# imulki/serenade

Hardware: AMD Instinct MI355X
Metric: mel frames/sec converted (UNet ODE + vocoder), 80x1024 (higher is better)
Workload: dtype f32

## Files before the change

### serenade_amd/csrc/resunit_f32.hip

```cpp
#include <hip/hip_runtime.h>

#include "common.h"
#include "conv_common.h"
#include "fastdiv.h"
#include "serenade_hip.h"

namespace {

constexpr int NTH = 512;

template <int C_>
struct UCfg {
  static constexpr int C = C_, CH = C / 32;
  static constexpr int BMI = C == 32 ? 256 : 128;
  static constexpr int A_ROWS = BMI + SRN_RESUNIT_HALO_MAX + 2;
  static constexpr int A_PLANE = A_ROWS * 144;
  static constexpr int A_BYTES = CH * A_PLANE;
  static constexpr int UNIT = C * 144;
  static constexpr int G = 9216 / UNIT >= 2 ? 2 : 1;
  static constexpr int STAGE = G * UNIT;
  static constexpr int SMEM = A_BYTES + 2 * STAGE;
  static constexpr int F4R = C / 4, RSTEP = NTH / F4R;
  static constexpr int A_LD = (A_ROWS * F4R + NTH - 1) / NTH;
  static_assert(G * C * 8 == NTH, "one 16-B weight piece per thread per stage");
};

template <class R>
__global__ __launch_bounds__(NTH, 4) void resunit_f32_kernel(const SrnResUnitParams p, const int tiles_per_z,
                                                             const int n_tiles, const FDiv d_tpz) {
  constexpr int C = R::C, CH = R::CH, BMI = R::BMI, G = R::G;
  extern __shared__ __attribute__((aligned(16))) unsigned char smem_u[];
  unsigned char* const sA = smem_u;
  unsigned char* const sW = smem_u + R::A_BYTES;

  const int tid = threadIdx.x;
  const int lane = tid & 63;
  const int wave = __builtin_amdgcn_readfirstlane(tid >> 6);
  const int li = lane & 31;
  const int lh = lane >> 5;
  const int k = p.k, dil = p.dilation, T = p.T;
  const int p2 = (k - 1) / 2, p1 = p2 * dil;
  const int BMo = BMI - (k - 1);
  const int hr = BMI + (k - 1) * dil;
  const int U = k * CH;
  const int S = (U + G - 1) / G;
  const float slope = p.slope;

  const int w_n = (tid % (C * 8)) >> 3;
  const int w_g = tid / (C * 8);
  const int w_voff = w_n * (k * C * 4) + w_g * 128 + (tid & 7) * 16;
  const int w_dst = (w_g * C + w_n) * 144 + (tid & 7) * 16;
  const int w_bytes = C * k * C * 4;
  const __amdgpu_buffer_rsrc_t rs_w1 = srn_buffer_rsrc(p.w1, w_bytes);
  const __amdgpu_buffer_rsrc_t rs_w2 = srn_buffer_rsrc(p.w2, w_bytes);
  u32x4 wr;
  auto w_load = [&](const int j) {
    if (j >= S) wr = __builtin_amdgcn_raw_buffer_load_b128(rs_w2, w_voff, (j - S) * G * 128, 0);
    else wr = __builtin_amdgcn_raw_buffer_load_b128(rs_w1, w_voff, j * G * 128, 0);
  };
  auto w_store = [&](const int buf) {
    *reinterpret_cast<u32x4*>(sW + buf * R::STAGE + w_dst) = wr;
  };

  constexpr int A_LD = R::A_LD, F4R = R::F4R, RSTEP = R::RSTEP;
  const int a_f4 = tid % F4R;
  const int a_r0 = tid / F4R;
  const int a_voff = (a_r0 * C + a_f4 * 4) * 4;
  const int a_dst0 = (a_f4 >> 3) * R::A_PLANE + a_r0 * 144 + (a_f4 & 7) * 16;
  u32x4 pa[A_LD];
  auto load_a = [&](const int tile) {
    const int z = fdiv(tile, d_tpz);
    const int t0 = (tile - z * tiles_per_z) * BMo;
    const __amdgpu_buffer_rsrc_t rs_x = srn_buffer_rsrc(p.x + (int64_t)z * p.x_bs, T * C * 4);
    const int v0 = a_voff + (t0 - p2 - p1) * (C * 4);
#pragma unroll
    for (int j = 0; j < A_LD; ++j) pa[j] = __builtin_amdgcn_raw_buffer_load_b128(rs_x, v0 + j * (RSTEP * C * 4), 0, 0);
  };
  auto stage_a = [&]() {
#pragma unroll
    for (int j = 0; j < A_LD; ++j) {
      if (a_r0 + RSTEP * j < hr) {
        float4 v = __builtin_bit_cast(float4, pa[j]);
        v.x = fmaxf(v.x, v.x * slope);
        v.y = fmaxf(v.y, v.y * slope);
        v.z = fmaxf(v.z, v.z * slope);
        v.w = fmaxf(v.w, v.w * slope);
        *reinterpret_cast<float4*>(sA + a_dst0 + j * RSTEP * 144) = v;
      }
    }
  };

  const int wm0 = (C == 64 ? (wave & 3) : wave) * 32;
  const int ng0 = C == 64 ? (wave >> 2) : 0;
  const int fa_lane = (wm0 + li) * 144 + 16 * lh;
  const int fb_lane = R::A_BYTES + (ng0 * 32 + li) * 144 + 16 * lh;
  f32x16 acc;
  auto zero_acc = [&]() {
#pragma unroll
    for (int r = 0; r < 16; ++r) acc[r] = 0.f;
  };

  auto compute = [&](const int buf, const int u0, const int step) {
#pragma unroll
    for (int g = 0; g < G; ++g) {
      const int u = u0 + g;
      if (u >= U) break;
      const int tap = u / CH;
      const int c = u - tap * CH;
      const float* a = reinterpret_cast<const float*>(smem_u + (fa_lane + (c * R::A_PLANE + tap * step * 144)));
      const float* b = reinterpret_cast<const float*>(smem_u + (fb_lane + (buf * R::STAGE + g * C * 144)));
#pragma unroll
      for (int kk = 0; kk < 4; ++kk) {
        const float4 af = *reinterpret_cast<const float4*>(a + kk * 8);
        const float4 bf = *reinterpret_cast<const float4*>(b + kk * 8);
        acc = __builtin_amdgcn_mfma_f32_32x32x2f32(af.x, bf.x, acc, 0, 0, 0);
        acc = __builtin_amdgcn_mfma_f32_32x32x2f32(af.y, bf.y, acc, 0, 0, 0);
        acc = __builtin_amdgcn_mfma_f32_32x32x2f32(af.z, bf.z, acc, 0, 0, 0);
        acc = __builtin_amdgcn_mfma_f32_32x32x2f32(af.w, bf.w, acc, 0, 0, 0);
      }
    }
  };

  int wj = 0, wbuf = 0;
  auto conv_pass = [&](const int step) {
    for (int s = 0; s < S; ++s) {
      compute(wbuf, s * G, step);
      w_store(wbuf ^ 1);
      int nxt = wj + 2;
      if (nxt >= 2 * S) nxt -= 2 * S;
      w_load(nxt);
      wj = wj + 1 == 2 * S ? 0 : wj + 1;
      wbuf ^= 1;
      __syncthreads();
    }
  };

  int tile = blockIdx.x;
  load_a(tile);
  w_load(0);
  w_store(0);
  w_load(2 * S > 1 ? 1 : 0);

  const float bias1 = p.b1[ng0 * 32 + li];
  const float bias2 = p.b2[ng0 * 32 + li];
  const bool divide = p.post_div != 0.f && p.post_div != 1.f;
  const bool has_q = p.res2 != nullptr;
  const int mid_lane = ng0 * R::A_PLANE + ((wm0 + 4 * lh) * 36 + li) * 4;
  const int io_lane = ((wm0 + 4 * lh) * C + ng0 * 32 + li) * 4;

  for (; tile < n_tiles; tile += gridDim.x) {
    const int z = fdiv(tile, d_tpz);
    const int t0 = (tile - z * tiles_per_z) * BMo;
    stage_a();
    __syncthreads();
    const int next = tile + gridDim.x;
    load_a(next < n_tiles ? next : tile);

    zero_acc();
    conv_pass(dil);
    if (t0 - p2 >= 0 && t0 - p2 + BMI <= T) {
#pragma unroll
      for (int r = 0; r < 16; ++r) {
        const float v = acc[r] + bias1;
        *reinterpret_cast<float*>(sA + mid_lane + ((r & 3) + 8 * (r >> 2)) * 144) = fmaxf(v, v * slope);
      }
    } else {
#pragma unroll
      for (int r = 0; r < 16; ++r) {
        const int dr = (r & 3) + 8 * (r >> 2);
        const int gi = t0 - p2 + wm0 + 4 * lh + dr;
        float v = acc[r] + bias1;
        v = fmaxf(v, v * slope);
        if (gi < 0 || gi >= T) v = 0.f;
        *reinterpret_cast<float*>(sA + mid_lane + dr * 144) = v;
      }
    }
    __syncthreads();

    zero_acc();
    conv_pass(1);

    const int row_end = min(BMo, T - t0);
    const int64_t zoff = (int64_t)t0 * C;
    const int io_bytes = row_end * C * 4;
    const __amdgpu_buffer_rsrc_t rs_xe = srn_buffer_rsrc(p.x + (int64_t)z * p.x_bs + zoff, io_bytes);
    const __amdgpu_buffer_rsrc_t rs_qe =
        srn_buffer_rsrc(has_q ? p.res2 + (int64_t)z * p.res2_bs + zoff : p.x, has_q ? io_bytes : 0);
    const __amdgpu_buffer_rsrc_t rs_oe = srn_buffer_rsrc(p.out + (int64_t)z * p.out_bs + zoff, io_bytes);
    if (wm0 + 32 <= row_end) {
#pragma unroll
      for (int gq = 0; gq < 4; ++gq) {
        float xv[4], qv[4];
#pragma unroll
        for (int i = 0; i < 4; ++i) {
          xv[i] = __builtin_bit_cast(float, __builtin_amdgcn_raw_buffer_load_b32(rs_xe, io_lane, (8 * gq + i) * C * 4, 0));
          qv[i] = __builtin_bit_cast(float, __builtin_amdgcn_raw_buffer_load_b32(rs_qe, io_lane, (8 * gq + i) * C * 4, 0));
        }
#pragma unroll
        for (int i = 0; i < 4; ++i) {
          float v = acc[4 * gq + i] + bias2 + xv[i];
          if (has_q) v += qv[i];
          if (divide) v = v / p.post_div;
          __builtin_amdgcn_raw_buffer_store_b32(__builtin_bit_cast(unsigned, v), rs_oe, io_lane, (8 * gq + i) * C * 4, 0);
        }
      }
    } else if (wm0 < row_end) {
#pragma unroll
      for (int gq = 0; gq < 4; ++gq) {
        float xv[4], qv[4];
#pragma unroll
        for (int i = 0; i < 4; ++i) {
          xv[i] = __builtin_bit_cast(float, __builtin_amdgcn_raw_buffer_load_b32(rs_xe, io_lane + (8 * gq + i) * C * 4, 0, 0));
          qv[i] = __builtin_bit_cast(float, __builtin_amdgcn_raw_buffer_load_b32(rs_qe, io_lane + (8 * gq + i) * C * 4, 0, 0));
        }
#pragma unroll
        for (int i = 0; i < 4; ++i) {
          float v = acc[4 * gq + i] + bias2 + xv[i];
          if (has_q) v += qv[i];
          if (divide) v = v / p.post_div;
          __builtin_amdgcn_raw_buffer_store_b32(__builtin_bit_cast(unsigned, v), rs_oe, io_lane + (8 * gq + i) * C * 4, 0, 0);
        }
      }
    }
  }
}

template <class R>
int launch_unit(const SrnResUnitParams& p, const SrnResUnitRoute& r, hipStream_t stream) {
  static SrnSmemAttr smem_attr;
  if (const int e = smem_attr.ensure(reinterpret_cast<const void*>(&resunit_f32_kernel<R>), R::SMEM)) return e;
  static_assert(R::BMI == srn_resunit_bmi(R::C), "the route's tile height is the kernel's");
  hipLaunchKernelGGL((resunit_f32_kernel<R>), dim3(r.grid), dim3(NTH), R::SMEM, stream, p, r.tiles_per_z, r.n_tiles,
                     make_fdiv((uint32_t)r.tiles_per_z));
  SRN_CHECK_LAUNCH();
  return 0;
}

}

bool srn_resunit_f32_eligible(const SrnResUnitParams& p, const SrnResUnitRoute& r) {
  if (!(p.slope >= 0.f && p.slope <= 1.f)) return false;
  if ((int64_t)p.T * p.C * 4 >= 0x7fffffffll) return false;
  return r.n_tiles < (1 << 26);
}

int srn_resunit_f32_launch(const SrnResUnitParams& p, const SrnResUnitRoute& r, hipStream_t stream) {
  return p.C == 32 ? launch_unit<UCfg<32>>(p, r, stream) : launch_unit<UCfg<64>>(p, r, stream);
}
```

Measured before the change: 62580.

## Process contiguous runs of subtiles per block, carrying halo rows in LDS

Each block now walks a contiguous run of time subtiles instead of independent strided tiles. It carries the k-1 halo rows of the mid activation between consecutive subtiles in shared memory, so after the first subtile it stops recomputing the overlapping first-conv rows. A host planner sizes the runs so that every batch fills the grid slots, and an env var can force the run length. The change adds index bookkeeping, a carry path and uneven run lengths, and it risks load imbalance or halo bugs at run boundaries.

```diff
diff --git a/serenade_amd/csrc/resunit_f32.hip b/serenade_amd/csrc/resunit_f32.hip
--- a/serenade_amd/csrc/resunit_f32.hip
+++ b/serenade_amd/csrc/resunit_f32.hip
@@ -1,4 +1,5 @@
 #include <hip/hip_runtime.h>
+#include <stdlib.h>
 
 #include "common.h"
 #include "conv_common.h"
@@ -25,9 +26,13 @@
   static_assert(G * C * 8 == NTH, "one 16-B weight piece per thread per stage");
 };
 
+struct Runs {
+  int n_sub, n_long, runs_per_z, z_flip, n_runs;
+  FDiv d_rpz;
+};
+
 template <class R>
-__global__ __launch_bounds__(NTH, 4) void resunit_f32_kernel(const SrnResUnitParams p, const int tiles_per_z,
-                                                             const int n_tiles, const FDiv d_tpz) {
+__global__ __launch_bounds__(NTH, 4) void resunit_f32_kernel(const SrnResUnitParams p, const Runs rn) {
   constexpr int C = R::C, CH = R::CH, BMI = R::BMI, G = R::G;
   extern __shared__ __attribute__((aligned(16))) unsigned char smem_u[];
   unsigned char* const sA = smem_u;
@@ -68,11 +73,9 @@
   const int a_voff = (a_r0 * C + a_f4 * 4) * 4;
   const int a_dst0 = (a_f4 >> 3) * R::A_PLANE + a_r0 * 144 + (a_f4 & 7) * 16;
   u32x4 pa[A_LD];
-  auto load_a = [&](const int tile) {
-    const int z = fdiv(tile, d_tpz);
-    const int t0 = (tile - z * tiles_per_z) * BMo;
+  auto load_a = [&](const int z, const int row0) {
     const __amdgpu_buffer_rsrc_t rs_x = srn_buffer_rsrc(p.x + (int64_t)z * p.x_bs, T * C * 4);
-    const int v0 = a_voff + (t0 - p2 - p1) * (C * 4);
+    const int v0 = a_voff + row0 * (C * 4);
 #pragma unroll
     for (int j = 0; j < A_LD; ++j) pa[j] = __builtin_amdgcn_raw_buffer_load_b128(rs_x, v0 + j * (RSTEP * C * 4), 0, 0);
   };
@@ -135,8 +138,22 @@
     }
   };
 
-  int tile = blockIdx.x;
-  load_a(tile);
+  const int n_runs = rn.n_runs;
+  const int run_rows = rn.n_sub * BMI - (k - 1);
+  auto place = [&](const int run, int& z, int& t0, int& left) {
+    z = fdiv(run, rn.d_rpz);
+    const int pos = run - z * rn.runs_per_z;
+    const int lo = z >= rn.z_flip ? rn.runs_per_z - rn.n_long : 0;
+    t0 = pos * run_rows + min(max(pos - lo, 0), rn.n_long) * BMI;
+    const int len = rn.n_sub + (pos >= lo && pos - lo < rn.n_long);
+    const int rest = T - t0 - BMo;
+    left = rest <= 0 ? 0 : min(len - 1, (rest + BMI - 1) / BMI);
+  };
+  int run = blockIdx.x;
+  int z, t0, left;
+  int sub = 0;
+  place(run, z, t0, left);
+  load_a(z, t0 - p2 - p1);
   w_load(0);
   w_store(0);
   w_load(2 * S > 1 ? 1 : 0);
@@ -148,39 +165,55 @@
   const int mid_lane = ng0 * R::A_PLANE + ((wm0 + 4 * lh) * 36 + li) * 4;
   const int io_lane = ((wm0 + 4 * lh) * C + ng0 * 32 + li) * 4;
 
-  for (; tile < n_tiles; tile += gridDim.x) {
-    const int z = fdiv(tile, d_tpz);
-    const int t0 = (tile - z * tiles_per_z) * BMo;
+  for (;;) {
+    const int m0 = sub == 0 ? t0 - p2 : t0 + p2;
+    const int mid_off = sub == 0 ? 0 : (k - 1) * 144;
+    const int rows_out = sub == 0 ? BMo : BMI;
+    const int c_lo = sub == 1 ? RSTEP - (k - 1) : 0;
+    const bool carries = sub != 0 && a_r0 >= c_lo && a_r0 < c_lo + (k - 1);
+    float4 carry;
+    if (carries) carry = *reinterpret_cast<const float4*>(sA + a_dst0 + (sub == 1 ? BMI - RSTEP : BMI) * 144);
     stage_a();
     __syncthreads();
-    const int next = tile + gridDim.x;
-    load_a(next < n_tiles ? next : tile);
+    int nrun = run, nz = z, nt0 = t0 + rows_out, nsub = sub + 1, nleft = left - 1;
+    if (left == 0) {
+      nrun = run + gridDim.x;
+      if (nrun < n_runs) {
+        place(nrun, nz, nt0, nleft);
+        nsub = 0;
+      } else {
+        nt0 = t0;
+        nsub = sub;
+      }
+    }
+    load_a(nz, nsub == 0 ? nt0 - p2 - p1 : nt0 + p2 - p1);
 
     zero_acc();
     conv_pass(dil);
-    if (t0 - p2 >= 0 && t0 - p2 + BMI <= T) {
+    if (m0 >= 0 && m0 + BMI <= T) {
 #pragma unroll
       for (int r = 0; r < 16; ++r) {
         const float v = acc[r] + bias1;
-        *reinterpret_cast<float*>(sA + mid_lane + ((r & 3) + 8 * (r >> 2)) * 144) = fmaxf(v, v * slope);
+        *reinterpret_cast<float*>(sA + mid_lane + mid_off + ((r & 3) + 8 * (r >> 2)) * 144) = fmaxf(v, v * slope);
       }
     } else {
 #pragma unroll
       for (int r = 0; r < 16; ++r) {
         const int dr = (r & 3) + 8 * (r >> 2);
-        const int gi = t0 - p2 + wm0 + 4 * lh + dr;
+        const int gi = m0 + wm0 + 4 * lh + dr;
         float v = acc[r] + bias1;
         v = fmaxf(v, v * slope);
         if (gi < 0 || gi >= T) v = 0.f;
-        *reinterpret_cast<float*>(sA + mid_lane + dr * 144) = v;
-      }
-    }
+        *reinterpret_cast<float*>(sA + mid_lane + mid_off + dr * 144) = v;
+      }
+    }
+    if (carries) *reinterpret_cast<float4*>(sA + a_dst0 - c_lo * 144) = carry;
     __syncthreads();
 
     zero_acc();
     conv_pass(1);
 
-    const int row_end = min(BMo, T - t0);
+    const int row_end = min(rows_out, T - t0);
     const int64_t zoff = (int64_t)t0 * C;
     const int io_bytes = row_end * C * 4;
     const __amdgpu_buffer_rsrc_t rs_xe = srn_buffer_rsrc(p.x + (int64_t)z * p.x_bs + zoff, io_bytes);
@@ -222,7 +255,32 @@
         }
       }
     }
+    if (left == 0 && nrun >= n_runs) break;
+    run = nrun, z = nz, t0 = nt0, sub = nsub, left = nleft;
   }
+}
+
+Runs plan_runs(const SrnResUnitParams& p, const SrnResUnitRoute& r, const int bmi, const int forced) {
+  const int k1 = p.k - 1;
+  Runs rn{1, 0, r.tiles_per_z, p.n_batch, 0, {}};
+  if (forced > 0) {
+    const int run_rows = forced * bmi - k1;
+    rn.n_sub = forced;
+    rn.runs_per_z = (p.T + run_rows - 1) / run_rows;
+  } else {
+    const int slots = r.grid / p.n_batch > 1 ? r.grid / p.n_batch : 1;
+    int n = (int)(((int64_t)p.T + (int64_t)slots * k1) / ((int64_t)slots * bmi));
+    if (n >= 2) {
+      const int64_t rest = p.T - (int64_t)slots * (n * bmi - k1);
+      int n_long = (int)((rest + bmi - 1) / bmi);
+      if (n_long == slots) ++n, n_long = 0;
+      rn.n_sub = n, rn.n_long = n_long, rn.runs_per_z = slots;
+      if (p.n_batch > 1) rn.z_flip = (p.n_batch + 1) / 2;
+    }
+  }
+  rn.n_runs = p.n_batch * rn.runs_per_z;
+  rn.d_rpz = make_fdiv((uint32_t)rn.runs_per_z);
+  return rn;
 }
 
 template <class R>
@@ -230,8 +288,16 @@
   static SrnSmemAttr smem_attr;
   if (const int e = smem_attr.ensure(reinterpret_cast<const void*>(&resunit_f32_kernel<R>), R::SMEM)) return e;
   static_assert(R::BMI == srn_resunit_bmi(R::C), "the route's tile height is the kernel's");
-  hipLaunchKernelGGL((resunit_f32_kernel<R>), dim3(r.grid), dim3(NTH), R::SMEM, stream, p, r.tiles_per_z, r.n_tiles,
-                     make_fdiv((uint32_t)r.tiles_per_z));
+  int forced = 0, grid_max = r.grid;
+  if (const char* e = getenv("SERENADE_AMD_RESUNIT_RUN")) {
+    const int got = sscanf(e, "%d,%d", &forced, &grid_max);
+    SRN_CHECK_ARG(got >= 1 && forced >= 1 && forced <= 64 && grid_max >= 1,
+                  "resunit: SERENADE_AMD_RESUNIT_RUN = \"%s\" (want n or n,grid with 1 <= n <= 64, grid >= 1)", e);
+    if (grid_max > r.grid) grid_max = r.grid;
+  }
+  const Runs rn = plan_runs(p, r, R::BMI, forced);
+  hipLaunchKernelGGL((resunit_f32_kernel<R>), dim3(rn.n_runs < grid_max ? rn.n_runs : grid_max), dim3(NTH), R::SMEM,
+                     stream, p, rn);
   SRN_CHECK_LAUNCH();
   return 0;
 }
```

Result: no change. 62510 (-0.1%).
